# MichaelVorndran/InconsistencyMasks

Measured on AMD Instinct MI355X. Metric: images/sec per IM generation (ensemble infer + IM build + 1 train epoch), 256x256, higher is better.
Workload: dtype f16; 1 GPU; ISIC-2018 binary 256x256x3, 2-model IM ensemble, tiny U-Net alpha=0.5 on MI355X (configs[1]); outputs=1, unlabeled_images=2335, unlabeled_images_per_gpu=2335, labeled_images=259, n_models=2, infer_batch=584, infer_batch_rule=functions.infer_batch_size: 584 at alpha<=0.5 else 128; short tail spread, train_batch_per_gpu=32, global_batch=32, parallelism=dp1, epoch_steps=80, kept=2307, train_images=2566

## Files before the change

### inconsistencymasks_amd/csrc/imk_conv.hip

```cpp
#include <cstdlib>
#include "imk_kernels.h"
#include "imk_elem.h"

#include "imk_stage.h"
#include "imk_switches.h"

#ifndef IMK_INF_WAVES
#define IMK_INF_WAVES 4
#endif
IMK_STAMP_TABLE(conv)
IMK_WGSTAMP_TABLE(conv)

namespace {


struct ImkConvGeom { int tiles_x, tiles_y, mt_total, nc8, nc8p, n_pass, ps, nsp; unsigned magic_tx, magic_pi; };
__host__ __device__ inline size_t imk_chain_w2_offset(size_t stage1_bytes, size_t out_bytes) {
    return ((stage1_bytes > out_bytes ? stage1_bytes : out_bytes) + 15) & ~(size_t)15;
}

template <int TH, int MT, int LM, bool CHAIN = false>
__device__ __forceinline__ void conv_mfma_body(const ImkConvArgs &a, const ImkConvGeom &gm, int bx, int by) {
    const int tiles_x = gm.tiles_x, tiles_y = gm.tiles_y, mt_total = gm.mt_total, nc8 = gm.nc8, nc8p = gm.nc8p;
    const int n_pass = gm.n_pass, ps = gm.ps, nsp = gm.nsp;
// ... 305 lines not shown
    conv_mfma_body<TH, MT, LM, CHAIN>(a, gm, blockIdx.x, blockIdx.y);
}

constexpr size_t pipe_lds_base(int nc8, bool pair, int wg) {
    size_t b = (size_t)18 * 18 * imk_lds_pitch(nc8) * 16 + (8 * 16 + 4 * 2 * 16) * sizeof(float) + 1024 +
               ((wg && wg != 4) ? (size_t)(wg == 3 ? 18 * 18 : 256) * ((pair ? 1 : 2) | 1) * 16 + 64 : 0);
    if (wg == 3 && b < 4 * 5 * 256 * sizeof(float)) b = 4 * 5 * 256 * sizeof(float);
    return (b + 15) & ~(size_t)15;
}

template <int LM, int NC8, int CHAIN, bool PAIR, int EPI, bool DYSTAT, bool FULL, int WG = 0, int PRE = 0, bool DYN = false>
__global__ __launch_bounds__(256, (DYN && NC8 == 1) ? IMK_INF_WAVES : 1) void conv_pipe_kernel(ImkConvArgs a, int tiles_x, int tiles_y, int n_tiles,
                                                        unsigned magic_tx, ImkWalk wk) {
    static_assert(!DYN || (EPI == EP_RELU && !DYSTAT && WG == 0), "dynamic walk: results must not depend on the tile -> workgroup map");
    static_assert(PRE == 0 || (WG == 0 && EPI == EP_RELU && !DYSTAT && (LM == LM_U8 || LM == LM_UPADD)), "pre-stage: inference forward only");
    static_assert(WG != 1 || (LM == LM_BNBWD && CHAIN == 0 && EPI == EP_MASK && !DYSTAT && FULL), "fused wgrad: 1x1 dgrad behind a BatchNorm");
    static_assert(WG != 2 || (LM == LM_RAW && CHAIN == 0 && EPI == EP_PLAIN && DYSTAT && FULL), "fused wgrad: 1x1 dgrad in front of a BatchNorm");
    static_assert(WG != 3 || (LM == LM_RAW && CHAIN == 0 && EPI == EP_PLAIN && DYSTAT && FULL), "fused wgrad: 3x3 dgrad in front of a BatchNorm");
    static_assert(WG != 4 || (LM == LM_BNBWD && CHAIN == 0 && EPI == EP_PLAIN && !DYSTAT && FULL && PRE == 0), "2x2-sum epilogue: 1x1 dgrad of a decoder's first conv");
    constexpr int P = PAIR ? 2 : 4;
    constexpr int PS = imk_lds_pitch(NC8);
    constexpr int NCI = PRE ? PRE : NC8;
    constexpr int PSI = imk_lds_pitch(NCI);
    constexpr int MAX_ITEMS = (18 * 18 * NCI + 255) / 256;
    constexpr int MAX_NS = PAIR ? 3 * NC8 : (9 * NC8 + 3) / 4;
    extern __shared__ __attribute__((aligned(16))) uint8_t smem[];
    const int ks3 = (a.ksize == 3);
    const int halo = ks3 ? 1 : 0;
    const int HT = 16 + 2 * halo, WT = TW + 2 * halo;
    const int n_items = HT * WT * NCI;
    const bool shared_taps = PAIR && ks3;
// ... 1509 lines not shown

constexpr int PIPE_BLOCKS_PER_CU = 8;

template <int LM, int NC8, int CHAIN, bool PAIR, int EPI, bool DYSTAT, bool FULL, int WG = 0, int PRE = 0, bool DYN = false>
static int launch_conv_pipe_k(const ImkConvArgs &a, hipStream_t stream) {
    if constexpr (!DYN && EPI == EP_RELU && !DYSTAT && WG == 0) {
        if (a.sched && !a.stats_partial && a.B * imk_cdiv(a.H, 16) * imk_cdiv(a.W, TW) >= 2048)
            return launch_conv_pipe_k<LM, NC8, CHAIN, PAIR, EPI, DYSTAT, FULL, WG, PRE, true>(a, stream);
    }
    if (a.x.cs_in != (PRE ? PRE : NC8) * 8) return IMK_EINVAL;
    static int blocks_per_cu = 0;
    const size_t lds = pipe_lds_base(NC8, PAIR, WG) + (PRE ? (size_t)18 * 18 * imk_lds_pitch(PRE) * 16 + 3 * 16 * sizeof(float) : 0);
    auto kern = conv_pipe_kernel<LM, NC8, CHAIN, PAIR, EPI, DYSTAT, FULL, WG, PRE, DYN>;
    if (blocks_per_cu == 0) {
        int nb = 0;
        if (hipOccupancyMaxActiveBlocksPerMultiprocessor(&nb, kern, 256, lds) != hipSuccess || nb < 1) nb = 4;
        blocks_per_cu = nb > PIPE_BLOCKS_PER_CU ? PIPE_BLOCKS_PER_CU : nb;
    }
    const int tiles_x = imk_cdiv(a.W, TW), tiles_y = imk_cdiv(a.H, 16);
    const int n_tiles = a.B * tiles_x * tiles_y;
    int grid = 256 * blocks_per_cu;
    if (grid > n_tiles) grid = n_tiles;
    const ImkWalk wk = imk_walk_make(grid, n_tiles, tiles_x * tiles_y, DYN);
    if (DYN && wk.shift != 5) return IMK_EINVAL;
    ImkProfScope prof(PF_CONV_PIPE, imk_conv_algorithmic_bytes(a), stream, imk_conv_flops(a));
    imk_klaunch(kern, dim3(grid), dim3(256), lds, stream, a, tiles_x, tiles_y, n_tiles, div_magic(tiles_x), wk);
    IMK_LAUNCH_CHECK();
    if (a.stats_rows) *a.stats_rows = grid;
    return IMK_OK;
}

// ... 35 lines not shown
            return launch_conv_pipe_k<LM_BNBWD, NC8, 0, PAIR, EP_PLAIN, false, true, 4>(a, stream);
        } else {
            return IMK_EUNSUPPORTED;
        }
    }
    if (a.wg_partial) {
        if constexpr (FULL) {
            const bool dys = a.dystat_z && a.stats_partial;
            if (a.ksize == 3) {
                if (a.x.lmode == LM_RAW && a.epi == EP_PLAIN && dys && a.wg_sc && a.wg_sh)
                    return launch_conv_pipe_k<LM_RAW, NC8, 0, PAIR, EP_PLAIN, true, true, 3>(a, stream);
                return IMK_EUNSUPPORTED;
            }
            if (a.x.lmode == LM_BNBWD && a.epi == EP_MASK && !dys)
                return launch_conv_pipe_k<LM_BNBWD, NC8, 0, PAIR, EP_MASK, false, true, 1>(a, stream);
            if (a.x.lmode == LM_RAW && a.epi == EP_PLAIN && dys && a.wg_sc && a.wg_sh)
                return launch_conv_pipe_k<LM_RAW, NC8, 0, PAIR, EP_PLAIN, true, true, 2>(a, stream);
            return IMK_EUNSUPPORTED;
        } else {
            return IMK_EUNSUPPORTED;
        }
    }
    const bool dystat = a.dystat_z && a.stats_partial;
#define IMK_PIPE_BWD(LM)                                                                                         \
    (a.epi == EP_MASK ? (dystat ? launch_conv_pipe_k<LM, NC8, 0, PAIR, EP_MASK, true, FULL>(a, stream)           \
                                : launch_conv_pipe_k<LM, NC8, 0, PAIR, EP_MASK, false, FULL>(a, stream))         \
                      : (dystat ? launch_conv_pipe_k<LM, NC8, 0, PAIR, EP_PLAIN, true, FULL>(a, stream)          \
                                : launch_conv_pipe_k<LM, NC8, 0, PAIR, EP_PLAIN, false, FULL>(a, stream)))
    switch (a.x.lmode) {
        case LM_RAW: return IMK_PIPE_BWD(LM_RAW);
// ... 152 lines not shown
        return true;
    if ((sw.gemm_over_chain == 2 || (sw.gemm_over_chain == 1 && store_mid)) && imk_conv_gemm_ok(plain)) return false;
    if (pipe_choice(a).ok || a.epi != EP_RELU || a.ksize != 3 || a.cout > 64 || cout2 > 64) return false;
    if (a.x.lmode != LM_POOL && a.x.lmode != LM_AFFINE) return false;
    const bool wide = a.x.cs_in <= 32 && a.cout <= 32 && a.x.lmode != LM_POOL;
    const bool wide_chain = sw.wide_chain_train && wide && a.x.lmode == LM_AFFINE && a.x.cs_in >= 16 && cout2 <= a.cout && pipe_fits(a);
    if (sw.conv_chain_tile == 1 && wide && store_mid && !wide_chain && (long long)a.B * imk_cdiv(a.H, 16) * imk_cdiv(a.W, TW) > 2048)
        return false;
    const int mt1 = (a.cout + 15) / 16, mt2 = (cout2 + 15) / 16, mt = (mt1 <= 2 && mt2 <= 2) ? 2 : 4;
    return mt1 <= mt && mt2 <= mt && conv_tile_h(a.x.cs_in, 3) == 16;
}

bool imk_conv_can_fuse_wgrad(const ImkConvArgs &a) {
    const PipeChoice p = pipe_choice(a);
    if (!p.ok || a.wpk2) return false;
    const bool form1 = a.ksize == 1 && a.x.lmode == LM_BNBWD && a.epi == EP_MASK && a.mask && !(a.dystat_z && a.stats_partial);
    const bool form2 = a.x.lmode == LM_RAW && a.epi == EP_PLAIN && a.dystat_z && a.stats_partial;
    if (!form1 && !form2) return false;
    const bool all_ch = p.pair ? a.cs_out == 8 : a.cs_out == 16;
    return (a.H % 16 == 0) && (a.W % TW == 0) && all_ch;
}
int imk_conv_fused_wgrad_rows_max() { return 256 * 8; }

bool imk_conv_can_sum2(const ImkConvArgs &a) {
    const PipeChoice p = pipe_choice(a);
    if (!p.ok || a.wpk2 || a.wg_partial) return false;
    if (a.ksize != 1 || a.x.lmode != LM_BNBWD || a.epi != EP_PLAIN || (a.dystat_z && a.stats_partial)) return false;
    const bool all_ch = p.pair ? a.cs_out == 8 : a.cs_out == 16;
    return (a.H % 16 == 0) && (a.W % TW == 0) && all_ch;
}

int imk_launch_conv(const ImkConvArgs &a_in, hipStream_t stream) {
    ImkConvArgs a = a_in;
    IMK_CHECK_ARG(a.x.in && a.wpk && (a.out || a.wpk2) && a.B > 0 && a.H > 0 && a.W > 0);
    IMK_CHECK_ARG(a.ksize == 1 || a.ksize == 3);
    IMK_CHECK_ARG(a.x.cs_in % 8 == 0 && a.cs_out % 8 == 0 && a.x.cs_in >= a.x.cin && a.cs_out >= a.cout);
    IMK_CHECK_ARG(a.x.lmode != LM_U8 || (a.x.cs_in == 8 && a.x.cin <= 8));
    if (a.x.cs_in > 512) return IMK_EUNSUPPORTED;
    const PipeChoice p = pipe_choice(a);
    a.pair = p.pair;
    if (a.pre_wpk && !(p.ok && a.wpk2 && a.pre_bias && a.pre_sc && a.pre_sh && a.pre_cout > 0)) return IMK_EUNSUPPORTED;
    if (a.wpk2 && a.pair && a.cout2 > 8) return IMK_EUNSUPPORTED;
    if (a.wpk2) {
        if (a.epi != EP_RELU || !a.out2 || !a.bias2 || a.cs_out2 % 8) return IMK_EUNSUPPORTED;
        if (p.ok) return a.cout2 > 16 ? IMK_EUNSUPPORTED : launch_conv_pipe_any(a, stream);
        if (!imk_conv_can_chain_tile(a, a.cout2, a.out != nullptr)) return IMK_EUNSUPPORTED;
        if (conv_wide_chain_ok(a)) return launch_conv_wide_chain(a, stream);
        if (imk_conv_gemm_chain_ok(a)) return imk_launch_conv_gemm(a, stream);
        return launch_conv_mfma(a, stream);
    }
    if (p.ok) return launch_conv_pipe_any(a, stream);
    if (a.x.lmode == LM_STEM) return IMK_EUNSUPPORTED;
    if (conv_wide_ok(a)) return launch_conv_wide_any(a, stream);
// ... 112 lines not shown
```

### inconsistencymasks_amd/csrc/imk_elem.h

```cpp
#pragma once
#include "imk_common.h"

struct ImkCtl {
    float loss_scale;
    float inv_loss_scale;
    int good_steps;
    int step;
    float found_inf;
    float pad[3];
};

int imk_launch_bn_finalize(const float *partial, int n_part, int c, int cs, double count, const float *gamma,
                           const float *beta, float *mov_mean, float *mov_var, float *scale, float *shift,
                           float *save_mean, float *save_invstd, hipStream_t stream, float momentum = 0.99f);
int imk_bn_prep_blocks(int B, int H, int W, int cs);
int imk_launch_bn_bwd_prep(int mode, const f16 *g_direct, const f16 *g_other, const f16 *z, const float *sc,
                           const float *sh, f16 *dy_out, float *partial, int B, int H, int W, int cs, hipStream_t stream,
                           int g_other_cs = 0);
int imk_launch_bn_bwd_coef(const float *partial, int n_part, int c, int cs, double count, const float *gamma,
                           const float *save_mean, const float *save_invstd, const float *inv_scale_ptr, float *coef,
                           float *dgamma, float *dbeta, float *found_inf, hipStream_t stream);
int imk_launch_head(const f16 *z, const float *sc, const float *sh, const float *w, const float *bias, int cin, int cs,
                    int K, int softmax, long long n_pix, float *probs, hipStream_t stream);
int imk_loss_blocks(long long n_pix);
int imk_launch_head_loss(const f16 *z, const float *sc, const float *sh, const float *w, const float *bias, int cin, int cs,
                         int K, int softmax, long long n_pix, const uint8_t *y, const ImkCtl *ctl, float *stats,
                         f16 *dlogit, float *loss_partial, hipStream_t stream);
bool imk_head_cce_fused_ok(int cs, int K, long long n_pix, int rows_cap);
int imk_head_cce_fused_rows(long long n_pix);
int imk_launch_head_cce_fused(const f16 *z, const float *sc, const float *sh, const float *w, const float *bias, int cin, int cs,
                              int K, long long n_pix, const uint8_t *y, const ImkCtl *ctl, float *stats, f16 *dy,
                              float *loss_partial, float *dystat_partial, float *wg_partial, hipStream_t stream);
bool imk_head_mse_fused_ok(int cs, int K, long long n_pix, int rows_cap);
int imk_launch_head_mse_fused(const f16 *z, const float *sc, const float *sh, const float *w, const float *bias, int cin, int cs,
                              int K, long long n_pix, const uint8_t *y, const ImkCtl *ctl, float *stats, f16 *dy,
                              float *loss_partial, float *dystat_partial, float *wg_partial, hipStream_t stream);
int imk_launch_loss_finalize(const float *loss_partial, long long n_pix, int K, int kind, float *stats, hipStream_t stream);
bool imk_consistency_fused_ok(int cs, int K, int softmax, long long n_pix, int rows_cap);
int imk_launch_consistency_head(const f16 *zA, const f16 *zB, const float *scA, const float *shA, const float *scB,
                                const float *shB, const float *w, const float *bias, int cin, int cs, int K, long long n_pix,
                                const ImkCtl *ctl, float *stats, f16 *dyA, f16 *dyB, float *loss_partial, float *dystatA,
                                float *dystatB, float *wg_partial, hipStream_t stream);
int imk_launch_consistency_dlogit(const float *pA, const float *pB, int K, int softmax, long long n_pix, const ImkCtl *ctl,
                                  float *stats, f16 *dlogitA, f16 *dlogitB, float *loss_partial, hipStream_t stream);
int imk_launch_grad_add(float *g, const float *g2, long long n, float *found_inf, hipStream_t stream);
int imk_launch_ctl_init(ImkCtl *ctl, hipStream_t stream);
int imk_launch_adamw(float *p, float *m, float *v, const float *g, long long n, ImkCtl *ctl, const float *stats,
                     float grad_scale, float lr, float wd, float b1, float b2, float eps, hipStream_t stream);

int imk_launch_concat_pool(const f16 *za, const float *sca, const float *sha, int csa, const f16 *zb, const float *scb,
                           const float *shb, int csb, int B, int Hh, int Wh, f16 *cat, hipStream_t stream, int a_div = 1);
// ... 25 lines not shown
```

### inconsistencymasks_amd/csrc/imk_headf.hip

```cpp
#include "imk_stage.h"

IMK_STAMP_TABLE(headf)

namespace {

struct HeadCceArgs {
    const f16 *z;
    const float *sc, *sh;
    const float *w, *bias;
    int cin, cs, K;
    long long n_pix;
    const uint8_t *y;
    const ImkCtl *ctl;
    float *stats;
    f16 *dy;
    float *loss_partial;
    float *dystat_partial;
    float *wg_partial;
    int cot_n;
};

template <int CS, int KT>
__global__ __launch_bounds__(256) void head_cce_fused_kernel(HeadCceArgs a) {
    IMK_STAMP_BEGIN(headf, 90001);
    constexpr int NCT = CS / 16;
    constexpr int NS = (KT + 1) / 2;
    constexpr int KT2 = 2 * NS;
    constexpr int H16 = WG_STRIDE_H;
    constexpr int IMG_H = (NCT + KT) * 64 * H16;
    extern __shared__ __attribute__((aligned(16))) uint8_t smem[];
    const int t = threadIdx.x, lane = t & 63, wave = t >> 6, p16 = lane & 15, g = lane >> 4, qq = p16 >> 2, pp = p16 & 3;
    f16 *s_x = reinterpret_cast<f16 *>(smem) + wave * IMG_H;
    f16 *s_g = s_x + NCT * 64 * H16;
    const int K = a.K, cin = a.cin;
// ... 211 lines not shown
        float v = 0.f;
        if (kt < KT) {
            if (tap == 0) {
                const int idx = (ct * KT + kt) * 256 + e;
                v = (s_red[idx] + s_red[NA * 256 + idx]) + (s_red[2 * NA * 256 + idx] + s_red[3 * NA * 256 + idx]);
            } else if (ct == 0 && e < 16) {
                const int idx = NCT * KT * 256 + kt * 64 + e;
                v = (s_red[idx] + s_red[NA * 256 + idx]) + (s_red[2 * NA * 256 + idx] + s_red[3 * NA * 256 + idx]);
            }
        }
        wp[i] = v;
    }
    IMK_STAMP_END(1);
}

template <int CS, int K>
__global__ __launch_bounds__(256) void head_mse_fused_kernel(HeadCceArgs a) {
    IMK_STAMP_BEGIN(headf, 90000);
    constexpr int NA = 2 * CS + CS * K + K + 1;
    __shared__ float s_w[K * CS], s_wd[K * CS], s_b[K], s_sc[CS], s_sh[CS];
    __shared__ float s_red[4][NA];
    const int t = threadIdx.x, lane = t & 63, wave = t >> 6;
    for (int i = t; i < K * CS; i += 256) {
        const int k = i / CS, c = i - k * CS;
        const float w = (c < a.cin) ? a.w[(size_t)c * K + k] : 0.f;
        s_w[i] = w;
        s_wd[i] = (float)(f16)w;
    }
    if (t < K) s_b[t] = a.bias[t];
    if (t < CS) { s_sc[t] = a.sc[t]; s_sh[t] = a.sh[t]; }
    const float S = a.ctl->loss_scale;
    if (blockIdx.x == 0 && t == 0) { a.stats[1] = 0.f; a.stats[2] = S; a.stats[3] = (float)a.ctl->step; }
// ... 23 lines not shown
        }
        f16x8 dv[CS / 8];
#pragma unroll
        for (int c = 0; c < CS; ++c) {
            float d = 0.f;
#pragma unroll
            for (int k = 0; k < K; ++k) {
                d += gk[k] * s_wd[k * CS + c];
                acc[2 * CS + c * K + k] += xin[c] * gk[k];
            }
            const f16 d16 = (f16)d;
            dv[c >> 3][c & 7] = d16;
            acc[c] += (float)d16;
            acc[CS + c] += (float)d16 * zf[c];
        }
#pragma unroll
        for (int q = 0; q < CS / 8; ++q) *reinterpret_cast<f16x8 *>(a.dy + p * CS + q * 8) = dv[q];
    };
    constexpr int NP = 4;
    long long p = (long long)blockIdx.x * 256 + t;
    for (; p + (NP - 1) * stride < a.n_pix; p += NP * stride) {
        f16x8 zz[NP][CS / 8];
        uint8_t yy[NP][K];
#pragma unroll
        for (int u = 0; u < NP; ++u)
#pragma unroll
            for (int q = 0; q < CS / 8; ++q) zz[u][q] = *reinterpret_cast<const f16x8 *>(a.z + (p + u * stride) * CS + q * 8);
#pragma unroll
        for (int u = 0; u < NP; ++u)
#pragma unroll
            for (int k = 0; k < K; ++k) yy[u][k] = a.y[(p + u * stride) * K + k];
#pragma unroll
// ... 23 lines not shown
        wp[t] = (ci < CS && co < K) ? tot(2 * CS + ci * K + co) : 0.f;
        wp[256 + t] = (t < K) ? tot(2 * CS + CS * K + t) : 0.f;
    }
    IMK_STAMP_END(1);
}

}

bool imk_head_mse_fused_ok(int cs, int K, long long n_pix, int rows_cap) {
    if (cs != 8 || K != 1) return false;
    return imk_loss_blocks(n_pix) <= rows_cap;
}

int imk_launch_head_mse_fused(const f16 *z, const float *sc, const float *sh, const float *w, const float *bias, int cin, int cs,
                              int K, long long n_pix, const uint8_t *y, const ImkCtl *ctl, float *stats, f16 *dy,
                              float *loss_partial, float *dystat_partial, float *wg_partial, hipStream_t stream) {
    HeadCceArgs a{z, sc, sh, w, bias, cin, cs, K, n_pix, y, ctl, stats, dy, loss_partial, dystat_partial, wg_partial, 1};
    const int grid = imk_loss_blocks(n_pix);
    ImkProfScope prof(PF_HEAD_LOSS, (double)n_pix * (cs * 2 + K + cs * 2), stream, 6.0 * n_pix * cin * K);
    if (cs == 8 && K == 1) imk_klaunch(head_mse_fused_kernel<8, 1>, dim3(grid), dim3(256), 0, stream, a);
    else return IMK_EUNSUPPORTED;
    IMK_LAUNCH_CHECK();
    return IMK_OK;
}

bool imk_head_cce_fused_ok(int cs, int K, long long n_pix, int rows_cap) {
    if ((cs != 8 && cs != 16 && cs != 24 && cs != 32) || K < 2 || K > 64) return false;
    return imk_loss_blocks(n_pix) <= rows_cap;
}

int imk_head_cce_fused_rows(long long n_pix) { return imk_loss_blocks(n_pix); }

int imk_launch_head_cce_fused(const f16 *z, const float *sc, const float *sh, const float *w, const float *bias, int cin, int cs,
                              int K, long long n_pix, const uint8_t *y, const ImkCtl *ctl, float *stats, f16 *dy,
                              float *loss_partial, float *dystat_partial, float *wg_partial, hipStream_t stream) {
// ... 17 lines not shown
```

### inconsistencymasks_amd/csrc/imk_kernels.h

```cpp
#pragma once
#include "imk_common.h"

enum ImkLoadMode {
    LM_RAW = 0,
    LM_AFFINE = 1,
    LM_POOL = 2,
    LM_UPADD = 3,
    LM_U8 = 4,
    LM_BNBWD = 5,
    LM_STEM = 6,
};
enum ImkEpilogue {
    EP_RELU = 0,
    EP_PLAIN = 1,
    EP_MASK = 2,
};

struct ImkInput {
    const void *in;
    const void *in2;
    const float *sc, *sh;
    const float *sc2, *sh2;
    int lmode;
    int cin, cs_in;
    float u8_div;
// ... 40 lines not shown
    return f;
}
bool imk_conv_can_fuse_wgrad(const ImkConvArgs &dgrad_args);
bool imk_conv_can_sum2(const ImkConvArgs &dgrad_args);
bool imk_conv_gemm_ok(const ImkConvArgs &a);
int imk_launch_conv_gemm(const ImkConvArgs &a, hipStream_t stream);
bool imk_conv_gemm_chain_ok(const ImkConvArgs &a);
int imk_conv_gemm_num_tiles(int B, int H, int W);
inline double imk_conv_algorithmic_bytes(const ImkConvArgs &a) {
    const double px = (double)a.B * a.H * a.W;
    double in_b;
    switch (a.x.lmode) {
        case LM_POOL: in_b = 4.0 * px * a.x.cs_in * 2; break;
        case LM_UPADD: in_b = px * a.x.cs_in * 2 + 0.25 * px * a.x.cs_in * 2; break;
        case LM_BNBWD: in_b = 2.0 * px * a.x.cs_in * 2; break;
        case LM_U8: in_b = px * a.x.cin; break;
        case LM_STEM: in_b = px * a.x.u8_c; break;
        default: in_b = px * a.x.cs_in * 2;
    }
    double out_b = (a.wpk2 && !a.out) ? 0.0 : px * a.cs_out * 2;
    if (a.wpk2) out_b += px * a.cs_out2 * 2;
    if (a.epi == EP_MASK) out_b += px * a.cs_out * 2;
    if (a.epi != EP_RELU && a.dystat_z) out_b += px * a.cs_out * 2;
    return in_b + out_b;
}
int imk_conv_fused_wgrad_rows_max();
int imk_conv_num_tiles(int B, int H, int W, int cs_in, int ksize);
int imk_launch_conv(const ImkConvArgs &a, hipStream_t stream);

struct ImkWgradArgs {
// ... 74 lines not shown
```

### inconsistencymasks_amd/csrc/imk_net.h

```cpp
#pragma once
#include <algorithm>
#include <cstdlib>
#include <cstring>
#include <mutex>
#include <new>
#include "imk_elem.h"
#include "imk_kernels.h"
#include "imk_plan.h"


namespace {

constexpr size_t ALIGN = 256;
inline size_t up(size_t v) { return (v + ALIGN - 1) / ALIGN * ALIGN; }

inline int add_conv(imk_unet_plan *p, const char *name, int k, int cin, int cout, int res) {
    ImkLayer l{};
    l.name = name; l.kind = 0; l.ksize = k; l.cin = cin; l.cout = cout; l.res = res;
    p->layers.push_back(l);
    return (int)p->layers.size() - 1;
}
inline int add_bn(imk_unet_plan *p, const char *name, int c, int res, int producer) {
    ImkLayer l{};
    l.name = name; l.kind = 1; l.ksize = 0; l.cin = c; l.cout = c; l.res = res; l.producer = producer;
// ... 243 lines not shown
    return StateView{(float *)b, (float *)(b + n), (ImkCtl *)(b + 2 * n)};
}

struct Bwd {
    Ctx &c;
    float *grads;
    ImkCtl *ctl;
    float *found_inf;
    int n_side;
    ImkWgFinalJobs jobs{};
    int n_fork = 0;
    bool used_side[imk_unet_plan::MAX_SIDE] = {};

    int dy_rows[64] = {};
    int sum2_bn = -1;

    void grad_input(int conv, ImkInput &in) const {
        const ImkLayer &l = c.p->layers[conv];
        in.cin = l.cout; in.cs_in = imk_pad8(l.cout);
        const int bn = l.bn_after;
        if (bn >= 0) {
            in.in = c.dy(bn); in.in2 = c.act(conv); in.lmode = LM_BNBWD;
            in.sc = reinterpret_cast<const float *>(c.base + c.ws.L[bn].coef);
        } else {
            in.in = c.dA(conv); in.lmode = LM_RAW;
        }
    }
    void dgrad_args(int conv, f16 *dst, const f16 *mask, int stat_bn, int *rows, ImkConvArgs &a) const {
        const ImkLayer &l = c.p->layers[conv];
        const Dim d = res_dim(c.p->cfg, l.res);
        grad_input(conv, a.x);
        a.B = c.B; a.H = d.h; a.W = d.w; a.ksize = l.ksize;
        a.cout = l.cin; a.cs_out = imk_pad8(l.cin);
        a.wpk = c.wbwd(conv);
        a.out = dst;
        a.mask = mask;
        a.epi = mask ? EP_MASK : EP_PLAIN;
        if (stat_bn >= 0) {
// ... 94 lines not shown
            hipEvent_t ev = c.p->ev_fork[n_fork++];
            IMK_HIP(hipEventRecord(ev, c.stream));
            IMK_HIP(hipStreamWaitEvent(ws, ev, 0));
        }
        used_side[si] = true;
        for (int i = 0; i < n_pending; ++i) {
            int rc = launch_wgrad(pending[i].conv, pending[i].dA_override, ws);
            if (rc) return rc;
        }
        n_pending = 0;
        if (defer_finalize) return IMK_OK;
        int rc = imk_launch_wgrad_finalize_jobs(jobs, &ctl->inv_loss_scale, found_inf, ws);
        jobs = ImkWgFinalJobs{};
        return rc;
    }
    int wgrad_dgrad(int conv, f16 *dst, const f16 *mask, int stat_bn = -1) {
        const int s2_bn = sum2_bn;
        sum2_bn = -1;
        const ImkLayer &l = c.p->layers[conv];
        if (mask && stat_bn < 0 && l.ksize == 1 && l.lmode == LM_RAW && l.src >= 0 && mask == c.act(l.src)) {
            ImkConvArgs a{};
            int rows = 0;
            dgrad_args(conv, dst, mask, -1, nullptr, a);
            if (imk_conv_can_fuse_wgrad(a)) {
                a.wg_partial = reinterpret_cast<float *>(c.base + c.ws.L[conv].wg_partial);
                a.stats_rows = &rows;
                int rc = imk_launch_conv(a, c.stream);
                if (rc) return rc;
                if (rows <= 0 || rows > imk_conv_fused_wgrad_rows_max()) return IMK_EWORKSPACE;
                return imk_wgf_add_job(jobs, a.wg_partial, rows, l.ksize, l.cin, l.cout, grads + l.off_w, grads + l.off_b);
            }
        }
        if (stat_bn < 0 && l.ksize == 1 && l.bn_after >= 0 && l.src >= 0 &&
            ((l.lmode == LM_RAW && mask && mask == c.act(l.src)) || (l.lmode == LM_UPADD && !mask)) &&
            imk_bwd1x1_ok(l.lmode, imk_pad8(l.cin), imk_pad8(l.cout), mask != nullptr)) {
            const Dim d = res_dim(c.p->cfg, l.res);
            const int rows = imk_bwd1x1_rows((long long)c.B * d.h * d.w, imk_pad8(l.cin), imk_pad8(l.cout));
            float *wgp = reinterpret_cast<float *>(c.base + c.ws.L[conv].wg_partial);
            const int bn = l.bn_after;
// ... 134 lines not shown
```

### inconsistencymasks_amd/csrc/imk_stage.h

```cpp
#pragma once
#include <cstdlib>
#include "imk_kernels.h"
#include "imk_elem.h"

typedef __attribute__((__vector_size__(4 * sizeof(__fp16)))) __fp16 h4;
#define LDS_PTR(T, p) ((__attribute__((address_space(3))) T *)(p))

namespace {

constexpr int TW = 16;
constexpr int WG_STRIDE_H = 16;
constexpr int WG_RED_CHUNK = 16;

__host__ __device__ constexpr int imk_lds_pitch(int nc8) { return nc8 <= 1 ? 1 : ((nc8 + 1) & ~3) + 2; }

struct TileCoord { int b, ty0, tx0; };

__device__ __forceinline__ TileCoord tile_coord(int tile, int tiles_x, int tiles_y, int th) {
    TileCoord c;
    const int per_img = tiles_x * tiles_y;
    c.b = tile / per_img;
    const int r = tile - c.b * per_img;
    const int ty = r / tiles_x;
    c.ty0 = ty * th;
// ... 76 lines not shown
            const uint8_t *p = (const uint8_t *)in.in + ((size_t)(b * H + y) * W + x) * in.cin;
            f16x8 o;
#pragma unroll
            for (int j = 0; j < 8; ++j) o[j] = (f16)(j < in.cin ? (float)p[j] / in.u8_div : 0.0f);
            return o;
        }
    }
}

__device__ __forceinline__ void stage_affine_table(const ImkInput &in, float *s_aff) {
    const int cs = in.cs_in;
    if (in.lmode == LM_AFFINE || in.lmode == LM_POOL || in.lmode == LM_UPADD)
        for (int i = threadIdx.x; i < cs; i += 256) { s_aff[i] = in.sc[i]; s_aff[cs + i] = in.sh[i]; }
    if (in.lmode == LM_UPADD)
        for (int i = threadIdx.x; i < cs; i += 256) { s_aff[2 * cs + i] = in.sc2[i]; s_aff[3 * cs + i] = in.sh2[i]; }
    if (in.lmode == LM_BNBWD)
        for (int i = threadIdx.x; i < 3 * cs; i += 256) s_aff[i] = in.sc[i];
    if (in.lmode == LM_STEM) {
        for (int i = threadIdx.x; i < cs; i += 256) {
            const bool real = i < in.cin;
            s_aff[i] = in.sc[i]; s_aff[cs + i] = in.sh[i];
            for (int c = 0; c < 4; ++c) s_aff[(2 + c) * cs + i] = (real && c < in.u8_c) ? (float)(f16)in.sc2[c * in.cin + i] : 0.f;
            s_aff[6 * cs + i] = real ? in.sh2[i] : 0.f;
        }
    }
}

template <int LM> struct RawChunk { f16x8 v[LM == LM_POOL ? 4 : ((LM == LM_UPADD || LM == LM_BNBWD) ? 2 : 1)]; };
template <> struct RawChunk<LM_U8> { uint32_t b[4]; };
template <> struct RawChunk<LM_STEM> { uint32_t b[4]; };

template <int LM>
__device__ __forceinline__ void raw_load(const ImkInput &in, int b, int y, int x, int H, int W, int c8, RawChunk<LM> &r) {
    const int cs = in.cs_in;
    if constexpr (LM == LM_RAW || LM == LM_AFFINE) {
        r.v[0] = *(const f16x8 *)((const f16 *)in.in + ((size_t)(b * H + y) * W + x) * cs + c8 * 8);
    } else if constexpr (LM == LM_POOL) {
        const int H2 = in.src_h ? in.src_h : 2 * H, W2 = in.src_w ? in.src_w : 2 * W;
        const f16 *p = (const f16 *)in.in + ((size_t)(b * H2 + 2 * y) * W2 + 2 * x) * cs + c8 * 8;
        r.v[0] = *(const f16x8 *)p;
        r.v[1] = *(const f16x8 *)(p + cs);
        r.v[2] = *(const f16x8 *)(p + (size_t)W2 * cs);
        r.v[3] = *(const f16x8 *)(p + (size_t)W2 * cs + cs);
    } else if constexpr (LM == LM_UPADD) {
        r.v[0] = *(const f16x8 *)((const f16 *)in.in + ((size_t)(b * (H / 2) + (y >> 1)) * (W / 2) + (x >> 1)) * cs + c8 * 8);
        r.v[1] = *(const f16x8 *)((const f16 *)in.in2 + ((size_t)(b * H + y) * W + x) * cs + c8 * 8);
    } else if constexpr (LM == LM_BNBWD) {
        const size_t o = ((size_t)(b * H + y) * W + x) * cs + c8 * 8;
        r.v[0] = *(const f16x8 *)((const f16 *)in.in + o);
        r.v[1] = *(const f16x8 *)((const f16 *)in.in2 + o);
    } else {
        const int nb = LM == LM_STEM ? in.u8_c : in.cin;
        const uint8_t *p = (const uint8_t *)in.in + ((size_t)(b * H + y) * W + x) * nb;
        typedef uint32_t __attribute__((aligned(1))) u32_unaligned;
        const int rem = (H * W - (y * W + x)) * nb;
        const int back = rem >= 4 ? 0 : 4 - rem;
        const uint32_t v = *reinterpret_cast<const u32_unaligned *>(p - back) >> (8 * back);
#pragma unroll
        for (int j = 0; j < 4; ++j) r.b[j] = (j < nb) ? ((v >> (8 * j)) & 0xffu) : 0u;
    }
}

template <int LM>
__device__ __forceinline__ f16x8 raw_transform(const RawChunk<LM> &r, const float *s_aff, int cs, int c8, int cin,
                                               float u8_div, int u8_c = 4) {
// ... 5 lines not shown
        return imk_affine_pool8(r.v[0], r.v[1], r.v[2], r.v[3], s_aff + c8 * 8, s_aff + cs + c8 * 8);
    } else if constexpr (LM == LM_UPADD) {
        const f16x8 lo = affine8(r.v[0], s_aff + c8 * 8, s_aff + cs + c8 * 8);
        const f16x8 sk = affine8(r.v[1], s_aff + 2 * cs + c8 * 8, s_aff + 3 * cs + c8 * 8);
        f16x8 o;
#pragma unroll
        for (int j = 0; j < 8; ++j) o[j] = (f16)((float)lo[j] + (float)sk[j]);
        return o;
    } else if constexpr (LM == LM_BNBWD) {
        const float *A = s_aff + c8 * 8, *Bc = s_aff + cs + c8 * 8, *Cc = s_aff + 2 * cs + c8 * 8;
        f16x8 o;
#pragma unroll
        for (int j = 0; j < 8; ++j) {
            const float zf = (float)r.v[1][j];
            o[j] = zf > 0.f ? (f16)(A[j] * (float)r.v[0][j] + Bc[j] * zf + Cc[j]) : (f16)0.f;
        }
        return o;
    } else if constexpr (LM == LM_STEM) {
        float xin[4];
#pragma unroll
        for (int c = 0; c < 4; ++c) xin[c] = (float)(f16)((float)r.b[c] * (1.0f / 255.0f));
        const float *sc = s_aff + c8 * 8, *sh = s_aff + cs + c8 * 8, *bias = s_aff + 6 * cs + c8 * 8;
        f16x8 o;
        float acc[8];
#pragma unroll
        for (int j = 0; j < 8; ++j) acc[j] = s_aff[2 * cs + c8 * 8 + j] * xin[0];
        if (u8_c > 1) {
#pragma unroll
            for (int j = 0; j < 8; ++j) acc[j] = fmaf(s_aff[4 * cs + c8 * 8 + j], xin[2], fmaf(s_aff[3 * cs + c8 * 8 + j], xin[1], acc[j]));
        }
// ... 73 lines not shown
    unsigned row2_b, w2, csb;
    int oy, ox, oyl, oxl, pix0, nb, hw, lo_y, hi_y, lo_x, hi_x;
};
template <int LM, unsigned CSB>
__device__ __forceinline__ PSrc<LM> psrc_of(const ImkInput &in, const PTile &tc, int halo, int HT, int WT, int H, int W) {
    PSrc<LM> s{};
    const int oy = tc.ty0 - halo, ox = tc.tx0 - halo;
    const unsigned csb = CSB ? CSB : (unsigned)in.cs_in * 2u;
    s.csb = csb;
    s.oy = oy; s.ox = ox;
    s.lo_y = oy < 0 ? -oy : 0; s.hi_y = min(HT - 1, H - 1 - oy);
    s.lo_x = ox < 0 ? -ox : 0; s.hi_x = min(WT - 1, W - 1 - ox);
    if constexpr (LM == LM_RAW || LM == LM_AFFINE || LM == LM_BNBWD) {
        s.b_in = pix_base(in.in, tc.b, H, W, oy, ox, csb);
        if constexpr (LM == LM_BNBWD) s.b_in2 = pix_base(in.in2, tc.b, H, W, oy, ox, csb);
    } else if constexpr (LM == LM_POOL) {
        const int H2 = in.src_h ? in.src_h : 2 * H, W2 = in.src_w ? in.src_w : 2 * W;
        s.b_in = pix_base(in.in, tc.b, H2, W2, 2 * oy, 2 * ox, csb);
        s.w2 = (unsigned)W2;
        s.row2_b = s.w2 * csb;
    } else if constexpr (LM == LM_UPADD) {
        s.oyl = oy >> 1; s.oxl = ox >> 1;
        s.b_in = pix_base(in.in, tc.b, H / 2, W / 2, s.oyl, s.oxl, csb);
        s.b_in2 = pix_base(in.in2, tc.b, H, W, oy, ox, csb);
    } else {
        s.nb = LM == LM_STEM ? in.u8_c : in.cin;
        s.hw = H * W;
        s.pix0 = oy * W + ox;
        s.b_in = reinterpret_cast<const char *>(in.in) + (long long)tc.b * s.hw * s.nb;
    }
    return s;
}
template <int LM, unsigned CSB>
__device__ __forceinline__ bool psrc_load(const PSrc<LM> &s, int py, int px, int c8, int W, RawChunk<LM> &r) {
    const int ry = min(max(py, s.lo_y), s.hi_y), rx = min(max(px, s.lo_x), s.hi_x);
    auto bytes = [&](unsigned pixels) { return CSB ? pixels * CSB : __umul24(pixels, s.csb); };
    if constexpr (LM == LM_RAW || LM == LM_AFFINE || LM == LM_BNBWD) {
        const unsigned o = bytes(__umul24(ry, W) + rx) + c8 * 16;
        r.v[0] = *reinterpret_cast<const f16x8 *>(s.b_in + o);
        if constexpr (LM == LM_BNBWD) r.v[1] = *reinterpret_cast<const f16x8 *>(s.b_in2 + o);
    } else if constexpr (LM == LM_POOL) {
        const unsigned o = bytes(__umul24(2 * ry, s.w2) + 2 * rx) + c8 * 16;
        r.v[0] = *reinterpret_cast<const f16x8 *>(s.b_in + o);
        r.v[1] = *reinterpret_cast<const f16x8 *>(s.b_in + o + s.csb);
        r.v[2] = *reinterpret_cast<const f16x8 *>(s.b_in + o + s.row2_b);
        r.v[3] = *reinterpret_cast<const f16x8 *>(s.b_in + o + s.row2_b + s.csb);
    } else if constexpr (LM == LM_UPADD) {
        const int yl = ((s.oy + ry) >> 1) - s.oyl, xl = ((s.ox + rx) >> 1) - s.oxl;
        r.v[0] = *reinterpret_cast<const f16x8 *>(s.b_in + bytes(__umul24(yl, W / 2) + xl) + c8 * 16);
        r.v[1] = *reinterpret_cast<const f16x8 *>(s.b_in2 + bytes(__umul24(ry, W) + rx) + c8 * 16);
    } else {
        typedef uint32_t __attribute__((aligned(1))) u32_unaligned;
        const int pidx = s.pix0 + (int)(__umul24(ry, W) + rx);
        const int rem = __mul24(s.hw - pidx, s.nb);
        const int back = rem >= 4 ? 0 : 4 - rem;
// ... 9 lines not shown
```

### inconsistencymasks_amd/csrc/imk_switches.cpp

```cpp
#include "imk_switches.h"
#include <cstdlib>
#include "imk_plan.h"

namespace {
bool on_unless_zero(const char *name) {
    const char *e = getenv(name);
    return !(e && e[0] == '0');
}
int int_or(const char *name, int dflt) {
    const char *e = getenv(name);
    return e ? atoi(e) : dflt;
}
}

const ImkSwitches &imk_switches() {
    static const ImkSwitches s = []() {
        ImkSwitches v{};
        v.conv_wide = on_unless_zero("IMK_CONV_WIDE");
        v.conv_gemm = on_unless_zero("IMK_CONV_GEMM");
        v.conv_chain_tile = int_or("IMK_CONV_CHAIN_TILE", 1);
        v.conv_prestage = on_unless_zero("IMK_CONV_PRESTAGE");
        v.wide_chain = on_unless_zero("IMK_WIDE_CHAIN");
        v.wide_chain_train = on_unless_zero("IMK_WIDE_CHAIN_TRAIN");
        v.gemm_chain = on_unless_zero("IMK_GEMM_CHAIN");
        v.gemm_over_chain = int_or("IMK_GEMM_OVER_CHAIN", 1);
        v.gemm_ad3_wgs = int_or("IMK_GEMM_AD3_WGS", 1024);
        v.wgrad_gemm_min = int_or("IMK_WGRAD_GEMM_MIN", 0);
        v.wgrad_nfo2 = on_unless_zero("IMK_WGRAD_NFO2");
        v.student_fused = on_unless_zero("IMK_STUDENT_FUSED");
        v.consistency_fused = on_unless_zero("IMK_CONSISTENCY_FUSED");
        v.select_shared = on_unless_zero("IMK_SELECT_SHARED");
        const int n = int_or("IMK_SIDE_STREAMS", 1);
        v.side_streams = n < 0 ? 0 : (n > imk_unet_plan::MAX_SIDE ? imk_unet_plan::MAX_SIDE : n);
        return v;
    }();
    return s;
}
```

### inconsistencymasks_amd/csrc/imk_switches.h

```cpp
#pragma once

struct ImkSwitches {
    bool conv_wide;
    bool conv_gemm;
    int conv_chain_tile;
    bool conv_prestage;
    bool wide_chain;
    bool wide_chain_train;
    bool gemm_chain;
    int gemm_over_chain;
    int gemm_ad3_wgs;
    int wgrad_gemm_min;
    bool wgrad_nfo2;
    bool student_fused;
    bool consistency_fused;
    bool select_shared;
    int side_streams;
};

const ImkSwitches &imk_switches();
```

### inconsistencymasks_amd/csrc/imk_unet.hip

```cpp
#include <atomic>
#include <cstdio>
#include "imk_net.h"
#include "imk_head.h"
#include "imk_switches.h"

namespace {


struct Topo {
    int in_c, in_bn;
    int e_c3[4], e_c1[4], e_bn[4];
    int b_c3, b_c1, b_bn;
    int d_ca[4], d_bna[4], d_c3[4], d_c1[4], d_bnb[4];
    int out;
};

Topo make_topo(const imk_unet_plan *p) {
    Topo t{};
    t.in_c = p->find("in.c"); t.in_bn = p->find("in.bn");
    char nm[16];
    for (int i = 0; i < 4; ++i) {
        snprintf(nm, sizeof nm, "e%d.c3", i + 1); t.e_c3[i] = p->find(nm);
        snprintf(nm, sizeof nm, "e%d.c1", i + 1); t.e_c1[i] = p->find(nm);
        snprintf(nm, sizeof nm, "e%d.bn", i + 1); t.e_bn[i] = p->find(nm);
// ... 664 lines not shown
    const int n_side = imk_switches().side_streams;
    const bool side_on = !plan->dbg_single_stream && n_side > 0 && ensure_side_streams(plan, n_side);
    Bwd b{c, grads, sv.ctl, stats + 1, side_on ? n_side : 0};
    ImkStopRingScope stop_ring(plan, stream, b.n_side);
    bool loss_done = false;
    auto loss_on_side = [&]() -> int {
        if (loss_done || b.n_side <= 0 || b.n_fork <= 0) return IMK_OK;
        loss_done = true;
        return imk_launch_loss_finalize(loss_partial, n_pix, cf.n_out, loss_kind, stats, plan->side[(b.n_fork - 1) % b.n_side]);
    };
    int head_rows = 0;
    HeadWgJob head_job{};
    if (head_mse_pass) {
        const int rows = imk_head_cce_fused_rows(n_pix);
        float *wgp = reinterpret_cast<float *>(c.base + c.ws.L[t.out].wg_partial);
        OK(imk_launch_head_mse_fused(c.act(t.d_c1[3]), c.bn_scale(obn), c.bn_shift(obn), params + ol.off_w, params + ol.off_b,
                                     ol.cin, imk_pad8(ol.cin), ol.cout, n_pix, y, sv.ctl, stats, c.dy(obn), loss_partial,
                                     reinterpret_cast<float *>(c.base + c.ws.L[obn].bwd_partial), wgp, stream));
        head_rows = rows;
        head_job = HeadWgJob{wgp, rows};
    } else if (head_one_pass) {
        const int rows = imk_head_cce_fused_rows(n_pix);
        float *wgp = reinterpret_cast<float *>(c.base + c.ws.L[t.out].wg_partial);
        OK(imk_launch_head_cce_fused(c.act(t.d_c1[3]), c.bn_scale(obn), c.bn_shift(obn), params + ol.off_w, params + ol.off_b,
                                     ol.cin, imk_pad8(ol.cin), ol.cout, n_pix, y, sv.ctl, stats, c.dy(obn), loss_partial,
                                     reinterpret_cast<float *>(c.base + c.ws.L[obn].bwd_partial), wgp, stream));
        head_rows = rows;
        head_job = HeadWgJob{wgp, rows};
    } else {
        OK(head_dgrad(b, t, dlogit, loss_on_side, &head_rows, &head_job));
    }
    OK(run_backward(b, t, head_rows, head_job.partial ? &head_job : nullptr, loss_on_side));
    if (!loss_done) OK(imk_launch_loss_finalize(loss_partial, n_pix, cf.n_out, loss_kind, stats, stream));
// ... 116 lines not shown
```

Baseline: 25660 images/s.

## Pass rank-1 head gradient to last decoder dgrad instead of full dy tensor

For the single-output MSE head, the fused head kernel now writes only the per-pixel scalar logit gradient instead of the full 8-channel dy tensor. The following 1x1 dgrad with fused wgrad reconstructs dy on load as g times the head weight vector through a new LM_BNBWD_R1 load mode. This cuts one write and one read of an 8-channel f16 activation per pixel in the training backward pass. The cost is extra load-mode plumbing and a slightly different rounding path, and it is gated by a switch and a fusion-eligibility probe.

```diff
diff --git a/inconsistencymasks_amd/csrc/imk_conv.hip b/inconsistencymasks_amd/csrc/imk_conv.hip
--- a/inconsistencymasks_amd/csrc/imk_conv.hip
+++ b/inconsistencymasks_amd/csrc/imk_conv.hip
@@ -343,7 +343,8 @@
                                                         unsigned magic_tx, ImkWalk wk) {
     static_assert(!DYN || (EPI == EP_RELU && !DYSTAT && WG == 0), "dynamic walk: results must not depend on the tile -> workgroup map");
     static_assert(PRE == 0 || (WG == 0 && EPI == EP_RELU && !DYSTAT && (LM == LM_U8 || LM == LM_UPADD)), "pre-stage: inference forward only");
-    static_assert(WG != 1 || (LM == LM_BNBWD && CHAIN == 0 && EPI == EP_MASK && !DYSTAT && FULL), "fused wgrad: 1x1 dgrad behind a BatchNorm");
+    static_assert(LM != LM_BNBWD_R1 || (WG == 1 && NC8 == 1 && PAIR), "rank-1 gradient on load: the last decoder block's 1x1 dgrad only");
+    static_assert(WG != 1 || ((LM == LM_BNBWD || LM == LM_BNBWD_R1) && CHAIN == 0 && EPI == EP_MASK && !DYSTAT && FULL), "fused wgrad: 1x1 dgrad behind a BatchNorm");
     static_assert(WG != 2 || (LM == LM_RAW && CHAIN == 0 && EPI == EP_PLAIN && DYSTAT && FULL), "fused wgrad: 1x1 dgrad in front of a BatchNorm");
     static_assert(WG != 3 || (LM == LM_RAW && CHAIN == 0 && EPI == EP_PLAIN && DYSTAT && FULL), "fused wgrad: 3x3 dgrad in front of a BatchNorm");
     static_assert(WG != 4 || (LM == LM_BNBWD && CHAIN == 0 && EPI == EP_PLAIN && !DYSTAT && FULL && PRE == 0), "2x2-sum epilogue: 1x1 dgrad of a decoder's first conv");
@@ -1883,7 +1884,8 @@
     auto kern = conv_pipe_kernel<LM, NC8, CHAIN, PAIR, EPI, DYSTAT, FULL, WG, PRE, DYN>;
     if (blocks_per_cu == 0) {
         int nb = 0;
-        if (hipOccupancyMaxActiveBlocksPerMultiprocessor(&nb, kern, 256, lds) != hipSuccess || nb < 1) nb = 4;
+        auto occ_kern = conv_pipe_kernel<(LM == LM_BNBWD_R1 ? (int)LM_BNBWD : LM), NC8, CHAIN, PAIR, EPI, DYSTAT, FULL, WG, PRE, DYN>;
+        if (hipOccupancyMaxActiveBlocksPerMultiprocessor(&nb, occ_kern, 256, lds) != hipSuccess || nb < 1) nb = 4;
         blocks_per_cu = nb > PIPE_BLOCKS_PER_CU ? PIPE_BLOCKS_PER_CU : nb;
     }
     const int tiles_x = imk_cdiv(a.W, TW), tiles_y = imk_cdiv(a.H, 16);
@@ -1949,6 +1951,10 @@
             }
             if (a.x.lmode == LM_BNBWD && a.epi == EP_MASK && !dys)
                 return launch_conv_pipe_k<LM_BNBWD, NC8, 0, PAIR, EP_MASK, false, true, 1>(a, stream);
+            if constexpr (NC8 == 1 && PAIR) {
+                if (a.x.lmode == LM_BNBWD_R1 && a.epi == EP_MASK && !dys && a.x.sc2)
+                    return launch_conv_pipe_k<LM_BNBWD_R1, 1, 0, true, EP_MASK, false, true, 1>(a, stream);
+            }
             if (a.x.lmode == LM_RAW && a.epi == EP_PLAIN && dys && a.wg_sc && a.wg_sh)
                 return launch_conv_pipe_k<LM_RAW, NC8, 0, PAIR, EP_PLAIN, true, true, 2>(a, stream);
             return IMK_EUNSUPPORTED;
@@ -2131,7 +2137,8 @@
 bool imk_conv_can_fuse_wgrad(const ImkConvArgs &a) {
     const PipeChoice p = pipe_choice(a);
     if (!p.ok || a.wpk2) return false;
-    const bool form1 = a.ksize == 1 && a.x.lmode == LM_BNBWD && a.epi == EP_MASK && a.mask && !(a.dystat_z && a.stats_partial);
+    const bool bnb = a.x.lmode == LM_BNBWD || (a.x.lmode == LM_BNBWD_R1 && a.x.cs_in == 8 && p.pair);
+    const bool form1 = a.ksize == 1 && bnb && a.epi == EP_MASK && a.mask && !(a.dystat_z && a.stats_partial);
     const bool form2 = a.x.lmode == LM_RAW && a.epi == EP_PLAIN && a.dystat_z && a.stats_partial;
     if (!form1 && !form2) return false;
     const bool all_ch = p.pair ? a.cs_out == 8 : a.cs_out == 16;
@@ -2154,6 +2161,7 @@
     IMK_CHECK_ARG(a.x.cs_in % 8 == 0 && a.cs_out % 8 == 0 && a.x.cs_in >= a.x.cin && a.cs_out >= a.cout);
     IMK_CHECK_ARG(a.x.lmode != LM_U8 || (a.x.cs_in == 8 && a.x.cin <= 8));
     if (a.x.cs_in > 512) return IMK_EUNSUPPORTED;
+    if (a.x.lmode == LM_BNBWD_R1 && !(a.wg_partial && imk_conv_can_fuse_wgrad(a))) return IMK_EUNSUPPORTED;
     const PipeChoice p = pipe_choice(a);
     a.pair = p.pair;
     if (a.pre_wpk && !(p.ok && a.wpk2 && a.pre_bias && a.pre_sc && a.pre_sh && a.pre_cout > 0)) return IMK_EUNSUPPORTED;
diff --git a/inconsistencymasks_amd/csrc/imk_elem.h b/inconsistencymasks_amd/csrc/imk_elem.h
--- a/inconsistencymasks_amd/csrc/imk_elem.h
+++ b/inconsistencymasks_amd/csrc/imk_elem.h
@@ -34,7 +34,8 @@
 bool imk_head_mse_fused_ok(int cs, int K, long long n_pix, int rows_cap);
 int imk_launch_head_mse_fused(const f16 *z, const float *sc, const float *sh, const float *w, const float *bias, int cin, int cs,
                               int K, long long n_pix, const uint8_t *y, const ImkCtl *ctl, float *stats, f16 *dy,
-                              float *loss_partial, float *dystat_partial, float *wg_partial, hipStream_t stream);
+                              float *loss_partial, float *dystat_partial, float *wg_partial, hipStream_t stream,
+                              f16 *g_rank1 = nullptr);
 int imk_launch_loss_finalize(const float *loss_partial, long long n_pix, int K, int kind, float *stats, hipStream_t stream);
 bool imk_consistency_fused_ok(int cs, int K, int softmax, long long n_pix, int rows_cap);
 int imk_launch_consistency_head(const f16 *zA, const f16 *zB, const float *scA, const float *shA, const float *scB,
diff --git a/inconsistencymasks_amd/csrc/imk_headf.hip b/inconsistencymasks_amd/csrc/imk_headf.hip
--- a/inconsistencymasks_amd/csrc/imk_headf.hip
+++ b/inconsistencymasks_amd/csrc/imk_headf.hip
@@ -18,6 +18,7 @@
     float *dystat_partial;
     float *wg_partial;
     int cot_n;
+    f16 *g;
 };
 
 template <int CS, int KT>
@@ -259,8 +260,9 @@
     IMK_STAMP_END(1);
 }
 
-template <int CS, int K>
+template <int CS, int K, bool R1 = false>
 __global__ __launch_bounds__(256) void head_mse_fused_kernel(HeadCceArgs a) {
+    static_assert(!R1 || K == 1, "rank-1 route: one sigmoid map");
     IMK_STAMP_BEGIN(headf, 90000);
     constexpr int NA = 2 * CS + CS * K + K + 1;
     __shared__ float s_w[K * CS], s_wd[K * CS], s_b[K], s_sc[CS], s_sh[CS];
@@ -314,8 +316,12 @@
             acc[c] += (float)d16;
             acc[CS + c] += (float)d16 * zf[c];
         }
-#pragma unroll
-        for (int q = 0; q < CS / 8; ++q) *reinterpret_cast<f16x8 *>(a.dy + p * CS + q * 8) = dv[q];
+        if constexpr (R1) {
+            a.g[p] = (f16)gk[0];
+        } else {
+#pragma unroll
+            for (int q = 0; q < CS / 8; ++q) *reinterpret_cast<f16x8 *>(a.dy + p * CS + q * 8) = dv[q];
+        }
     };
     constexpr int NP = 4;
     long long p = (long long)blockIdx.x * 256 + t;
@@ -369,11 +375,12 @@
 
 int imk_launch_head_mse_fused(const f16 *z, const float *sc, const float *sh, const float *w, const float *bias, int cin, int cs,
                               int K, long long n_pix, const uint8_t *y, const ImkCtl *ctl, float *stats, f16 *dy,
-                              float *loss_partial, float *dystat_partial, float *wg_partial, hipStream_t stream) {
-    HeadCceArgs a{z, sc, sh, w, bias, cin, cs, K, n_pix, y, ctl, stats, dy, loss_partial, dystat_partial, wg_partial, 1};
+                              float *loss_partial, float *dystat_partial, float *wg_partial, hipStream_t stream, f16 *g_rank1) {
+    HeadCceArgs a{z, sc, sh, w, bias, cin, cs, K, n_pix, y, ctl, stats, dy, loss_partial, dystat_partial, wg_partial, 1, g_rank1};
     const int grid = imk_loss_blocks(n_pix);
-    ImkProfScope prof(PF_HEAD_LOSS, (double)n_pix * (cs * 2 + K + cs * 2), stream, 6.0 * n_pix * cin * K);
-    if (cs == 8 && K == 1) imk_klaunch(head_mse_fused_kernel<8, 1>, dim3(grid), dim3(256), 0, stream, a);
+    ImkProfScope prof(PF_HEAD_LOSS, (double)n_pix * (cs * 2 + K + (g_rank1 ? 2 : cs * 2)), stream, 6.0 * n_pix * cin * K);
+    if (cs == 8 && K == 1 && g_rank1) imk_klaunch(head_mse_fused_kernel<8, 1, true>, dim3(grid), dim3(256), 0, stream, a);
+    else if (cs == 8 && K == 1) imk_klaunch(head_mse_fused_kernel<8, 1>, dim3(grid), dim3(256), 0, stream, a);
     else return IMK_EUNSUPPORTED;
     IMK_LAUNCH_CHECK();
     return IMK_OK;
diff --git a/inconsistencymasks_amd/csrc/imk_kernels.h b/inconsistencymasks_amd/csrc/imk_kernels.h
--- a/inconsistencymasks_amd/csrc/imk_kernels.h
+++ b/inconsistencymasks_amd/csrc/imk_kernels.h
@@ -9,6 +9,7 @@
     LM_U8 = 4,
     LM_BNBWD = 5,
     LM_STEM = 6,
+    LM_BNBWD_R1 = 7,
 };
 enum ImkEpilogue {
     EP_RELU = 0,
@@ -79,6 +80,7 @@
         case LM_POOL: in_b = 4.0 * px * a.x.cs_in * 2; break;
         case LM_UPADD: in_b = px * a.x.cs_in * 2 + 0.25 * px * a.x.cs_in * 2; break;
         case LM_BNBWD: in_b = 2.0 * px * a.x.cs_in * 2; break;
+        case LM_BNBWD_R1: in_b = px * a.x.cs_in * 2 + px * 2; break;
         case LM_U8: in_b = px * a.x.cin; break;
         case LM_STEM: in_b = px * a.x.u8_c; break;
         default: in_b = px * a.x.cs_in * 2;
diff --git a/inconsistencymasks_amd/csrc/imk_net.h b/inconsistencymasks_amd/csrc/imk_net.h
--- a/inconsistencymasks_amd/csrc/imk_net.h
+++ b/inconsistencymasks_amd/csrc/imk_net.h
@@ -7,6 +7,7 @@
 #include "imk_elem.h"
 #include "imk_kernels.h"
 #include "imk_plan.h"
+#include "imk_switches.h"
 
 
 namespace {
@@ -281,6 +282,9 @@
 
     int dy_rows[64] = {};
     int sum2_bn = -1;
+    int r1_conv = -1;
+    const f16 *r1_g = nullptr;
+    const float *r1_w = nullptr;
 
     void grad_input(int conv, ImkInput &in) const {
         const ImkLayer &l = c.p->layers[conv];
@@ -289,6 +293,7 @@
         if (bn >= 0) {
             in.in = c.dy(bn); in.in2 = c.act(conv); in.lmode = LM_BNBWD;
             in.sc = reinterpret_cast<const float *>(c.base + c.ws.L[bn].coef);
+            if (conv == r1_conv) { in.in = r1_g; in.sc2 = r1_w; in.lmode = LM_BNBWD_R1; }
         } else {
             in.in = c.dA(conv); in.lmode = LM_RAW;
         }
@@ -413,15 +418,20 @@
         jobs = ImkWgFinalJobs{};
         return rc;
     }
+    bool fuse1_args(int conv, f16 *dst, const f16 *mask, int stat_bn, ImkConvArgs &a) const {
+        const ImkLayer &l = c.p->layers[conv];
+        if (!(mask && stat_bn < 0 && l.ksize == 1 && l.lmode == LM_RAW && l.src >= 0 && mask == c.act(l.src))) return false;
+        dgrad_args(conv, dst, mask, -1, nullptr, a);
+        return imk_conv_can_fuse_wgrad(a);
+    }
     int wgrad_dgrad(int conv, f16 *dst, const f16 *mask, int stat_bn = -1) {
         const int s2_bn = sum2_bn;
         sum2_bn = -1;
         const ImkLayer &l = c.p->layers[conv];
-        if (mask && stat_bn < 0 && l.ksize == 1 && l.lmode == LM_RAW && l.src >= 0 && mask == c.act(l.src)) {
+        {
             ImkConvArgs a{};
             int rows = 0;
-            dgrad_args(conv, dst, mask, -1, nullptr, a);
-            if (imk_conv_can_fuse_wgrad(a)) {
+            if (fuse1_args(conv, dst, mask, stat_bn, a)) {
                 a.wg_partial = reinterpret_cast<float *>(c.base + c.ws.L[conv].wg_partial);
                 a.stats_rows = &rows;
                 int rc = imk_launch_conv(a, c.stream);
diff --git a/inconsistencymasks_amd/csrc/imk_stage.h b/inconsistencymasks_amd/csrc/imk_stage.h
--- a/inconsistencymasks_amd/csrc/imk_stage.h
+++ b/inconsistencymasks_amd/csrc/imk_stage.h
@@ -114,8 +114,10 @@
         for (int i = threadIdx.x; i < cs; i += 256) { s_aff[i] = in.sc[i]; s_aff[cs + i] = in.sh[i]; }
     if (in.lmode == LM_UPADD)
         for (int i = threadIdx.x; i < cs; i += 256) { s_aff[2 * cs + i] = in.sc2[i]; s_aff[3 * cs + i] = in.sh2[i]; }
-    if (in.lmode == LM_BNBWD)
+    if (in.lmode == LM_BNBWD || in.lmode == LM_BNBWD_R1)
         for (int i = threadIdx.x; i < 3 * cs; i += 256) s_aff[i] = in.sc[i];
+    if (in.lmode == LM_BNBWD_R1)
+        for (int i = threadIdx.x; i < cs; i += 256) s_aff[3 * cs + i] = i < in.cin ? (float)(f16)in.sc2[i] : 0.f;
     if (in.lmode == LM_STEM) {
         for (int i = threadIdx.x; i < cs; i += 256) {
             const bool real = i < in.cin;
@@ -129,6 +131,7 @@
 template <int LM> struct RawChunk { f16x8 v[LM == LM_POOL ? 4 : ((LM == LM_UPADD || LM == LM_BNBWD) ? 2 : 1)]; };
 template <> struct RawChunk<LM_U8> { uint32_t b[4]; };
 template <> struct RawChunk<LM_STEM> { uint32_t b[4]; };
+template <> struct RawChunk<LM_BNBWD_R1> { f16x8 z; f16 g; };
 
 template <int LM>
 __device__ __forceinline__ void raw_load(const ImkInput &in, int b, int y, int x, int H, int W, int c8, RawChunk<LM> &r) {
@@ -149,6 +152,10 @@
         const size_t o = ((size_t)(b * H + y) * W + x) * cs + c8 * 8;
         r.v[0] = *(const f16x8 *)((const f16 *)in.in + o);
         r.v[1] = *(const f16x8 *)((const f16 *)in.in2 + o);
+    } else if constexpr (LM == LM_BNBWD_R1) {
+        const size_t px = (size_t)(b * H + y) * W + x;
+        r.g = ((const f16 *)in.in)[px];
+        r.z = *(const f16x8 *)((const f16 *)in.in2 + px * cs + c8 * 8);
     } else {
         const int nb = LM == LM_STEM ? in.u8_c : in.cin;
         const uint8_t *p = (const uint8_t *)in.in + ((size_t)(b * H + y) * W + x) * nb;
@@ -184,6 +191,17 @@
         for (int j = 0; j < 8; ++j) {
             const float zf = (float)r.v[1][j];
             o[j] = zf > 0.f ? (f16)(A[j] * (float)r.v[0][j] + Bc[j] * zf + Cc[j]) : (f16)0.f;
+        }
+        return o;
+    } else if constexpr (LM == LM_BNBWD_R1) {
+        const float *A = s_aff + c8 * 8, *Bc = s_aff + cs + c8 * 8, *Cc = s_aff + 2 * cs + c8 * 8, *wd = s_aff + 3 * cs + c8 * 8;
+        const float gf = (float)r.g;
+        f16x8 o;
+#pragma unroll
+        for (int j = 0; j < 8; ++j) {
+            const float zf = (float)r.z[j];
+            const f16 dy = (f16)(0.f + gf * wd[j]);
+            o[j] = zf > 0.f ? (f16)(__builtin_fmaf(A[j], (float)dy, Bc[j] * zf) + Cc[j]) : (f16)0.f;
         }
         return o;
     } else if constexpr (LM == LM_STEM) {
@@ -287,6 +305,9 @@
     if constexpr (LM == LM_RAW || LM == LM_AFFINE || LM == LM_BNBWD) {
         s.b_in = pix_base(in.in, tc.b, H, W, oy, ox, csb);
         if constexpr (LM == LM_BNBWD) s.b_in2 = pix_base(in.in2, tc.b, H, W, oy, ox, csb);
+    } else if constexpr (LM == LM_BNBWD_R1) {
+        s.b_in = pix_base(in.in, tc.b, H, W, oy, ox, 2u);
+        s.b_in2 = pix_base(in.in2, tc.b, H, W, oy, ox, csb);
     } else if constexpr (LM == LM_POOL) {
         const int H2 = in.src_h ? in.src_h : 2 * H, W2 = in.src_w ? in.src_w : 2 * W;
         s.b_in = pix_base(in.in, tc.b, H2, W2, 2 * oy, 2 * ox, csb);
@@ -312,6 +333,10 @@
         const unsigned o = bytes(__umul24(ry, W) + rx) + c8 * 16;
         r.v[0] = *reinterpret_cast<const f16x8 *>(s.b_in + o);
         if constexpr (LM == LM_BNBWD) r.v[1] = *reinterpret_cast<const f16x8 *>(s.b_in2 + o);
+    } else if constexpr (LM == LM_BNBWD_R1) {
+        const unsigned pix = __umul24(ry, W) + rx;
+        r.g = *reinterpret_cast<const f16 *>(s.b_in + pix * 2u);
+        r.z = *reinterpret_cast<const f16x8 *>(s.b_in2 + bytes(pix) + c8 * 16);
     } else if constexpr (LM == LM_POOL) {
         const unsigned o = bytes(__umul24(2 * ry, s.w2) + 2 * rx) + c8 * 16;
         r.v[0] = *reinterpret_cast<const f16x8 *>(s.b_in + o);
diff --git a/inconsistencymasks_amd/csrc/imk_switches.cpp b/inconsistencymasks_amd/csrc/imk_switches.cpp
--- a/inconsistencymasks_amd/csrc/imk_switches.cpp
+++ b/inconsistencymasks_amd/csrc/imk_switches.cpp
@@ -30,6 +30,7 @@
         v.student_fused = on_unless_zero("IMK_STUDENT_FUSED");
         v.consistency_fused = on_unless_zero("IMK_CONSISTENCY_FUSED");
         v.select_shared = on_unless_zero("IMK_SELECT_SHARED");
+        v.head_rank1 = on_unless_zero("IMK_HEAD_RANK1");
         const int n = int_or("IMK_SIDE_STREAMS", 1);
         v.side_streams = n < 0 ? 0 : (n > imk_unet_plan::MAX_SIDE ? imk_unet_plan::MAX_SIDE : n);
         return v;
diff --git a/inconsistencymasks_amd/csrc/imk_switches.h b/inconsistencymasks_amd/csrc/imk_switches.h
--- a/inconsistencymasks_amd/csrc/imk_switches.h
+++ b/inconsistencymasks_amd/csrc/imk_switches.h
@@ -15,6 +15,7 @@
     bool student_fused;
     bool consistency_fused;
     bool select_shared;
+    bool head_rank1;
     int side_streams;
 };
 
diff --git a/inconsistencymasks_amd/csrc/imk_unet.hip b/inconsistencymasks_amd/csrc/imk_unet.hip
--- a/inconsistencymasks_amd/csrc/imk_unet.hip
+++ b/inconsistencymasks_amd/csrc/imk_unet.hip
@@ -702,9 +702,17 @@
     if (head_mse_pass) {
         const int rows = imk_head_cce_fused_rows(n_pix);
         float *wgp = reinterpret_cast<float *>(c.base + c.ws.L[t.out].wg_partial);
+        if (imk_switches().head_rank1 && ol.cout == 1) {
+            b.r1_conv = t.d_c1[3]; b.r1_g = dlogit; b.r1_w = params + ol.off_w;
+            ImkConvArgs probe{};
+            if (!b.fuse1_args(t.d_c1[3], c.dA(t.d_c3[3]), c.act(t.d_c3[3]), -1, probe) || probe.x.lmode != LM_BNBWD_R1) {
+                b.r1_conv = -1; b.r1_g = nullptr; b.r1_w = nullptr;
+            }
+        }
         OK(imk_launch_head_mse_fused(c.act(t.d_c1[3]), c.bn_scale(obn), c.bn_shift(obn), params + ol.off_w, params + ol.off_b,
                                      ol.cin, imk_pad8(ol.cin), ol.cout, n_pix, y, sv.ctl, stats, c.dy(obn), loss_partial,
-                                     reinterpret_cast<float *>(c.base + c.ws.L[obn].bwd_partial), wgp, stream));
+                                     reinterpret_cast<float *>(c.base + c.ws.L[obn].bwd_partial), wgp, stream,
+                                     b.r1_conv >= 0 ? dlogit : nullptr));
         head_rows = rows;
         head_job = HeadWgJob{wgp, rows};
     } else if (head_one_pass) {
```

Result: no change. 25730 images/s (median of 3 runs) (+0.3%).
